# BBischof/ESRecsys

Measured on AMD Instinct MI355X. Metric: training pairs/sec, higher is better.
Workload: dtype f32; 1 GPU; inbatch: V=1000000 x D=128 fp32 tables, B=8192, sparse Adagrad; score_precision=auto -> f16x2, ids=uniform, parallelism=single

## Files before the change

### esrecsys_amd/csrc/esr_optim.hip

```cpp
#include "esr_common.h"
#include "esr_adam.h"
#include "esr_inbatch_mfma.h"
#include "esr_segment.h"

#include <algorithm>

namespace esr {

enum SegOp { kAdagrad = 0, kSgd = 1, kToDense = 2, kMomentum = 3, kMomentumStep = 4, kMomentumStepLazy = 5, kAdamStepLazy = 6 };
struct NoSegExtra {};
struct MomentumArgs {
  float momentum;
};
struct MomentumLazyArgs {
  float momentum;
  int32_t* last[2];
  int now;
};
template <int OP> struct SegExtraT { using type = NoSegExtra; };
template <> struct SegExtraT<kMomentumStep> { using type = MomentumArgs; };
template <> struct SegExtraT<kMomentumStepLazy> { using type = MomentumLazyArgs; };
template <> struct SegExtraT<kAdamStepLazy> { using type = AdamLazyArgs; };

template <int VEC, int NCH>
__device__ __forceinline__ void param_load(RowRegs<VEC, NCH>& r, const void* table, int dtype, int64_t row, int D,
                                           int lig, int G, int nvec) {
  if (dtype == ESR_F32) {
    row_load(r, (const float*)table + row * D, lig, G, nvec);
  } else {
    const uint16_t* p = (const uint16_t*)table + row * D;
#pragma unroll
    for (int k = 0; k < NCH; ++k) {
      const int c = lig + k * G;
      if (c < nvec) {
        if constexpr (VEC == 4) {
          const uint2 u = *reinterpret_cast<const uint2*>(p + 4 * c);
          r.v[k][0] = __uint_as_float(u.x << 16);
          r.v[k][1] = __uint_as_float(u.x & 0xffff0000u);
          r.v[k][2] = __uint_as_float(u.y << 16);
          r.v[k][3] = __uint_as_float(u.y & 0xffff0000u);
        } else {
          r.v[k][0] = bf16_to_f32(p[c]);
        }
      } else {
#pragma unroll
        for (int e = 0; e < VEC; ++e) r.v[k][e] = 0.f;
      }
    }
  }
}

template <int VEC, int NCH>
__device__ __forceinline__ void param_store(const RowRegs<VEC, NCH>& r, void* table, int dtype, int64_t row, int D,
                                            int lig, int G, int nvec) {
  if (dtype == ESR_F32) {
    row_store(r, (float*)table + row * D, lig, G, nvec);
  } else {
    uint16_t* p = (uint16_t*)table + row * D;
#pragma unroll
    for (int k = 0; k < NCH; ++k) {
      const int c = lig + k * G;
      if (c < nvec) {
        if constexpr (VEC == 4) {
          uint2 u;
          u.x = (uint32_t)f32_to_bf16(r.v[k][0]) | ((uint32_t)f32_to_bf16(r.v[k][1]) << 16);
          u.y = (uint32_t)f32_to_bf16(r.v[k][2]) | ((uint32_t)f32_to_bf16(r.v[k][3]) << 16);
          *reinterpret_cast<uint2*>(p + 4 * c) = u;
        } else {
          p[c] = f32_to_bf16(r.v[k][0]);
        }
      }
    }
  }
}

__device__ __forceinline__ void momentum_step_elem(float& p, float& t, float g, float lr, float m) {
#pragma clang fp contract(off)
  t = g + m * t;
  p = p - lr * t;
}

template <int VEC, int NCH, int OP>
__device__ __forceinline__ void seg_apply(const FusedTables& ft, int dtype, int32_t vid, const RowRegs<VEC, NCH>& g,
                                          int D, int lig, int G, int nvec, float lr, float eps,
                                          const typename SegExtraT<OP>::type& ex) {
  void* table = ft.table[0];
  float* accum = ft.accum[0];
  int64_t base = ft.row_offset[0];
#pragma unroll
  for (int k = 1; k < kMaxFusedTables; ++k)
    if (k < ft.n && (int64_t)vid >= ft.row_offset[k]) {
      table = ft.table[k];
      accum = ft.accum[k];
      base = ft.row_offset[k];
    }
  const int64_t id = (int64_t)vid - base;
  const bool second = 1 < ft.n && (int64_t)vid >= ft.row_offset[1];
  if constexpr (OP == kToDense) {
    row_store(g, (float*)table + id * D, lig, G, nvec);
  } else if constexpr (OP == kAdamStepLazy) {
    float* nu = second ? ex.nu[1] : ex.nu[0];
    int32_t* last = second ? ex.last[1] : ex.last[0];
    RowRegs<VEC, NCH> w, a, b;
    row_load(w, (const float*)table + id * D, lig, G, nvec);
    row_load(a, accum + id * D, lig, G, nvec);
    row_load(b, nu + id * D, lig, G, nvec);
    adam_catchup(w, a, b, last[id], ex.now - 1, ex, lig, G);
    const float omb1 = 1.0f - ex.b1, omb2 = 1.0f - ex.b2;
    const int64_t V = (second ? ft.row_offset[2] : ft.row_offset[1]) - base;
#pragma unroll
    for (int k = 0; k < NCH; ++k)
#pragma unroll
      for (int e = 0; e < VEC; ++e) {
        if (VEC == 1 && adam_is_tail(id * D + lig + k * G, V, D))
          adam_elem_tail(w.v[k][e], a.v[k][e], b.v[k][e], g.v[k][e], ex.lr, ex.b1, ex.b2, omb1, omb2, ex.eps, ex.ibc1[0],
                         ex.ibc2[0]);
        else
          adam_elem(w.v[k][e], a.v[k][e], b.v[k][e], g.v[k][e], ex.lr, ex.b1, ex.b2, omb1, omb2, ex.eps, ex.ibc1[0],
                    ex.ibc2[0]);
      }
    row_store(w, (float*)table + id * D, lig, G, nvec);
    row_store(a, accum + id * D, lig, G, nvec);
    row_store(b, nu + id * D, lig, G, nvec);
    if (lig == 0) last[id] = ex.now;
  } else {
    constexpr bool kLazy = OP == kMomentumStepLazy, kState = OP != kSgd;
    int32_t* last = nullptr;
    int steps = 0;
    if constexpr (kLazy) {
      last = second ? ex.last[1] : ex.last[0];
      steps = ex.now - 1 - last[id];
    }
    RowRegs<VEC, NCH> w, a;
    param_load(w, table, dtype, id, D, lig, G, nvec);
    if constexpr (kState) row_load(a, accum + id * D, lig, G, nvec);
    DecayCoef dk{};
    if constexpr (kLazy) dk = decay_coef(steps, ex.momentum);
#pragma unroll
    for (int k = 0; k < NCH; ++k)
#pragma unroll
      for (int e = 0; e < VEC; ++e) {
        float& p = w.v[k][e];
        const float gv = g.v[k][e];
        if constexpr (OP == kSgd) {
          p -= lr * gv;
        } else if constexpr (OP == kMomentum) {
          a.v[k][e] += gv;
          p -= lr * gv;
        } else if constexpr (OP == kAdagrad) {
          adagrad_elem(p, a.v[k][e], gv, lr, eps);
        } else {
          if constexpr (kLazy)
            if (steps > 0) decay_apply(p, a.v[k][e], dk, lr, ex.momentum);
          momentum_step_elem(p, a.v[k][e], gv, lr, ex.momentum);
        }
      }
    if constexpr (kState) row_store(a, accum + id * D, lig, G, nvec);
    param_store(w, table, dtype, id, D, lig, G, nvec);
    if constexpr (kLazy)
      if (lig == 0) last[id] = ex.now;
  }
}

template <int VEC, int NCH, int OP>
__global__ __launch_bounds__(kBlock) void segment_update_kernel(FusedTables ft, int dtype, int D, int G,
                                                               const int32_t* __restrict__ sorted_ids,
                                                               const int32_t* __restrict__ perm, int64_t n,
                                                               float* __restrict__ grad_rows, float lr, float eps,
                                                               typename SegExtraT<OP>::type ex) {
  const int lig = threadIdx.x & (G - 1);
  const int64_t gpb = kBlock / G;
  const int64_t group = (int64_t)blockIdx.x * gpb + threadIdx.x / G;
  const int64_t ngroups = (int64_t)gridDim.x * gpb;
  const int nvec = D / VEC;
  const int64_t per = (n + ngroups - 1) / ngroups;
  const int64_t p_end = min(n, (group + 1) * per);
  for (int64_t p = group * per; p < p_end; ++p) {
    const int32_t id = sorted_ids[p];
    const bool head = p == 0 || sorted_ids[p - 1] != id;
    if (!head && ((p & (kSegChunk - 1)) != 0 || sorted_ids[p - kSegChunk] != id)) continue;
    const int64_t stop = min(head ? ((p + 2 * kSegChunk - 1) / kSegChunk) * kSegChunk : p + kSegChunk, n);
    RowRegs<VEC, NCH> g;
    row_load(g, grad_rows + (int64_t)perm[p] * D, lig, G, nvec);
    int64_t q = p + 1, e_run = p + 1;
    bool run_over = false;
    while (e_run < stop) {
      if (sorted_ids[e_run] != id) {
        run_over = true;
        break;
      }
      ++e_run;
    }
    for (; q + 4 <= e_run; q += 4) {
      RowRegs<VEC, NCH> t0, t1, t2, t3;
      row_load(t0, grad_rows + (int64_t)perm[q] * D, lig, G, nvec);
      row_load(t1, grad_rows + (int64_t)perm[q + 1] * D, lig, G, nvec);
      row_load(t2, grad_rows + (int64_t)perm[q + 2] * D, lig, G, nvec);
      row_load(t3, grad_rows + (int64_t)perm[q + 3] * D, lig, G, nvec);
#pragma unroll
      for (int k = 0; k < NCH; ++k)
#pragma unroll
        for (int e = 0; e < VEC; ++e) g.v[k][e] = (((g.v[k][e] + t0.v[k][e]) + t1.v[k][e]) + t2.v[k][e]) + t3.v[k][e];
    }
    for (; q < e_run; ++q) {
      RowRegs<VEC, NCH> t;
      row_load(t, grad_rows + (int64_t)perm[q] * D, lig, G, nvec);
#pragma unroll
      for (int k = 0; k < NCH; ++k)
#pragma unroll
        for (int e = 0; e < VEC; ++e) g.v[k][e] += t.v[k][e];
    }
    const bool ends = run_over || q == n || sorted_ids[q] != id;
    if (head && ends)
      seg_apply<VEC, NCH, OP>(ft, dtype, id, g, D, lig, G, nvec, lr, eps, ex);
    else
      row_store(g, grad_rows + (int64_t)perm[p] * D, lig, G, nvec);
  }
}

template <int VEC, int NCH, int OP>
__global__ __launch_bounds__(kBlock) void segment_long_kernel(FusedTables ft, int dtype, int D, int G,
                                                             const int32_t* __restrict__ sorted_ids,
                                                             const int32_t* __restrict__ perm, int64_t n,
                                                             const float* __restrict__ grad_rows, float lr,
                                                             float eps, typename SegExtraT<OP>::type ex) {
  __shared__ float red[kBlock * VEC * NCH];
  constexpr int kPass = 4;
  __shared__ long long s_long[kPass];
  __shared__ int s_nlong, s_hoff;
  const int tid = threadIdx.x, lig = tid & (G - 1), gidx = tid / G, NG = kBlock / G;
  const int nvec = D / VEC;
  const int64_t nbound = (n - 1) / kSegChunk;
  for (int64_t b0 = (int64_t)blockIdx.x * kPass; b0 < nbound; b0 += (int64_t)gridDim.x * kPass) {
    __syncthreads();
    if (tid == 0) s_nlong = 0;
    __syncthreads();
    {
      const int64_t B = (b0 + tid + 1) * kSegChunk;
      if (tid < kPass && b0 + tid < nbound) {
        const int32_t id_b = sorted_ids[B];
        const bool first = B < 2 * kSegChunk || sorted_ids[B - 2 * kSegChunk] != id_b;
        if (sorted_ids[B - kSegChunk] == id_b && first) s_long[atomicAdd(&s_nlong, 1)] = B;
      }
    }
    __syncthreads();
    const int nlong = s_nlong;
    for (int li = 0; li < nlong; ++li) {
      const int64_t nxt = s_long[li];
      const int32_t id = sorted_ids[nxt];
      const int64_t win = max<int64_t>(nxt - 2 * kSegChunk + 1, 0);
      if (tid < 64) {
        const int64_t pos = win + tid;
        const bool is_head = pos <= nxt - kSegChunk && sorted_ids[pos] == id && (pos == 0 || sorted_ids[pos - 1] != id);
        const unsigned long long m = __ballot(is_head);
        if (tid == 0) s_hoff = __ffsll((long long)m) - 1;
      }
      __syncthreads();
      const int64_t h = win + s_hoff;
      int64_t K = 0;
      for (int64_t k0 = 0;; k0 += kBlock) {
        const int64_t pos = nxt + (k0 + tid) * kSegChunk;
        const int cnt = __syncthreads_count(pos < n && sorted_ids[pos] == id);
        K += cnt;
        if (cnt < kBlock) break;
      }
      RowRegs<VEC, NCH> acc;
#pragma unroll
      for (int k = 0; k < NCH; ++k)
#pragma unroll
        for (int e = 0; e < VEC; ++e) acc.v[k][e] = 0.f;
      auto part_row = [&](int64_t i) { return (int64_t)perm[i == 0 ? h : nxt + (i - 1) * kSegChunk] * D; };
      int64_t i = gidx;
      for (; i + 3 * NG <= K; i += 4 * NG) {
        RowRegs<VEC, NCH> t0, t1, t2, t3;
        row_load(t0, grad_rows + part_row(i), lig, G, nvec);
        row_load(t1, grad_rows + part_row(i + NG), lig, G, nvec);
        row_load(t2, grad_rows + part_row(i + 2 * NG), lig, G, nvec);
        row_load(t3, grad_rows + part_row(i + 3 * NG), lig, G, nvec);
#pragma unroll
        for (int k = 0; k < NCH; ++k)
#pragma unroll
          for (int e = 0; e < VEC; ++e)
            acc.v[k][e] = (((acc.v[k][e] + t0.v[k][e]) + t1.v[k][e]) + t2.v[k][e]) + t3.v[k][e];
      }
      for (; i <= K; i += NG) {
        RowRegs<VEC, NCH> t;
        row_load(t, grad_rows + part_row(i), lig, G, nvec);
#pragma unroll
        for (int k = 0; k < NCH; ++k)
#pragma unroll
          for (int e = 0; e < VEC; ++e) acc.v[k][e] += t.v[k][e];
      }
#pragma unroll
      for (int k = 0; k < NCH; ++k)
#pragma unroll
        for (int e = 0; e < VEC; ++e) red[((gidx * G + lig) * NCH + k) * VEC + e] = acc.v[k][e];
      __syncthreads();
      if (gidx == 0) {
        const int used = (int)min<int64_t>(NG, K + 1);
        for (int gg = 1; gg < used; ++gg)
#pragma unroll
          for (int k = 0; k < NCH; ++k)
#pragma unroll
            for (int e = 0; e < VEC; ++e) acc.v[k][e] += red[((gg * G + lig) * NCH + k) * VEC + e];
        seg_apply<VEC, NCH, OP>(ft, dtype, id, acc, D, lig, G, nvec, lr, eps, ex);
      }
      __syncthreads();
    }
  }
}

__global__ __launch_bounds__(kBlock) void gather_rows_multi_kernel(FusedTables ft, int nchunk, int G,
                                                                  const int32_t* __restrict__ vids, int64_t n,
                                                                  uint4* __restrict__ out) {
  const int lig = threadIdx.x & (G - 1);
  const int64_t gpb = kBlock / G;
  const int64_t group = (int64_t)blockIdx.x * gpb + threadIdx.x / G;
  const int64_t ngroups = (int64_t)gridDim.x * gpb;
  for (int64_t r = group; r < n; r += ngroups) {
    const int64_t vid = vids[r];
    const uint4* table = reinterpret_cast<const uint4*>(ft.table[0]);
    int64_t base = ft.row_offset[0];
#pragma unroll
    for (int k = 1; k < kMaxFusedTables; ++k)
      if (k < ft.n && vid >= ft.row_offset[k]) {
        table = reinterpret_cast<const uint4*>(ft.table[k]);
        base = ft.row_offset[k];
      }
    const uint4* src = table + (vid - base) * nchunk;
    for (int c = lig; c < nchunk; c += G) out[r * nchunk + c] = src[c];
  }
}

struct IdSegments {
  const int32_t* ids[kMaxFusedTables];
  int64_t start[kMaxFusedTables + 1];
  int64_t offset[kMaxFusedTables];
  int n;
};
__global__ __launch_bounds__(kBlock) void concat_offset_ids_kernel(IdSegments sg, int32_t* __restrict__ out) {
  const int64_t total = sg.start[sg.n];
  for (int64_t i = (int64_t)blockIdx.x * kBlock + threadIdx.x; i < total; i += (int64_t)gridDim.x * kBlock) {
    const int32_t* src = sg.ids[0];
    int64_t start = 0, off = sg.offset[0];
#pragma unroll
    for (int k = 1; k < kMaxFusedTables; ++k)
      if (k < sg.n && i >= sg.start[k]) {
        src = sg.ids[k];
        start = sg.start[k];
        off = sg.offset[k];
      }
    out[i] = (int32_t)((int64_t)src[i - start] + off);
  }
}

template <int OP>
static int launch_segment_tables(const char* who, const FusedTables& ft, int dtype, int D, const int32_t* sorted_ids,
                                 const int32_t* perm, int64_t n, float* grad_rows, float lr, float eps,
                                 hipStream_t st, bool skip_long = false,
                                 typename SegExtraT<OP>::type ex = {}) {
  const RowGeom g = row_geom(D);
  if (g.nch > kMaxChunksPerLane) {
    set_error("%s: D=%d not supported", who, D);
    return ESR_EINVAL;
  }
  const int grid = grid_for_groups(n, g.G);
  const int grid2 = (int)std::min<int64_t>(kMaxGrid, cdiv(cdiv(n, kSegChunk), 4));
  ESR_DISPATCH_ROW(g, {
    ESR_KT("segment_update_kernel", st, hipLaunchKernelGGL((segment_update_kernel<VEC, NCH, OP>), dim3(grid), dim3(kBlock), 0, st, ft, dtype, D, g.G,
                       sorted_ids, perm, n, grad_rows, lr, eps, ex));
    if (n > kSegChunk && !skip_long)
      ESR_KT("segment_long_kernel", st, hipLaunchKernelGGL((segment_long_kernel<VEC, NCH, OP>), dim3(grid2), dim3(kBlock), 0, st, ft, dtype, D, g.G,
                         sorted_ids, perm, n, (const float*)grad_rows, lr, eps, ex));
  });
  return check_launch(who);
}

template <class T>
static int fused_tables(const char* who, FusedTables& ft, T* const* tables, float* const* states,
                        const int64_t* row_offsets, int ntables, bool strict = false, int max_tables = kMaxFusedTables) {
  ESR_REQUIRE(ntables >= 1 && ntables <= max_tables, "%s: ntables=%d not in [1, %d]", who, ntables, max_tables);
  ESR_REQUIRE(tables && row_offsets, "%s: null pointer", who);
  ft.n = ntables;
  for (int i = 0; i < kMaxFusedTables; ++i) {
    ft.table[i] = i < ntables ? const_cast<void*>((const void*)tables[i]) : nullptr;
    ft.accum[i] = i < ntables && states ? states[i] : nullptr;
    ft.row_offset[i] = row_offsets[std::min(i, ntables)];
    if (i < ntables) {
      ESR_REQUIRE(tables[i] || states, "%s: null table %d", who, i);
      ESR_REQUIRE(tables[i] && (!states || states[i]) && row_offsets[i + 1] >= row_offsets[i] + (strict ? 1 : 0),
                  "%s: bad table %d", who, i);
    }
  }
  ft.row_offset[kMaxFusedTables] = row_offsets[ntables];
  ESR_REQUIRE(row_offsets[ntables] < ((int64_t)1 << 31), "%s: %lld virtual rows >= 2^31", who, (long long)row_offsets[ntables]);
  return ESR_OK;
}

template <int OP>
static int launch_segment_update(const char* who, void* table, int dtype, float* accum, int D,
                                 const int32_t* sorted_ids, const int32_t* perm, int64_t n, float* grad_rows,
                                 float lr, float eps, hipStream_t st, typename SegExtraT<OP>::type ex = {}) {
  const int64_t row_offsets[2] = {0, 0};
  FusedTables ft;
  if (const int rc = fused_tables(who, ft, &table, accum ? &accum : nullptr, row_offsets, 1)) return rc;
  return launch_segment_tables<OP>(who, ft, dtype, D, sorted_ids, perm, n, grad_rows, lr, eps, st, false, ex);
}

__global__ __launch_bounds__(kBlock) void dense_adam_kernel(float* __restrict__ p, float* __restrict__ mu,
                                                           float* __restrict__ nu, const float* __restrict__ g,
                                                           int64_t n4, int64_t numel, float lr, float b1, float b2,
                                                           float eps, float inv_bc1, float inv_bc2) {
  const float omb1 = 1.0f - b1, omb2 = 1.0f - b2;
  auto upd = [&](float& pv, float& m, float& v, float gv) {
    adam_elem(pv, m, v, gv, lr, b1, b2, omb1, omb2, eps, inv_bc1, inv_bc2);
  };
  const int64_t stride = (int64_t)gridDim.x * kBlock;
  for (int64_t i = (int64_t)blockIdx.x * kBlock + threadIdx.x; i < n4; i += stride) {
    float4 pv = reinterpret_cast<float4*>(p)[i];
    float4 m = reinterpret_cast<float4*>(mu)[i];
    float4 v = reinterpret_cast<float4*>(nu)[i];
    const float4 gv = reinterpret_cast<const float4*>(g)[i];
    upd(pv.x, m.x, v.x, gv.x);
    upd(pv.y, m.y, v.y, gv.y);
    upd(pv.z, m.z, v.z, gv.z);
    upd(pv.w, m.w, v.w, gv.w);
    reinterpret_cast<float4*>(p)[i] = pv;
    reinterpret_cast<float4*>(mu)[i] = m;
    reinterpret_cast<float4*>(nu)[i] = v;
  }
  for (int64_t i = n4 * 4 + (int64_t)blockIdx.x * kBlock + threadIdx.x; i < numel; i += stride) {
    float pv = p[i], m = mu[i], v = nu[i];
    adam_elem_tail(pv, m, v, g[i], lr, b1, b2, omb1, omb2, eps, inv_bc1, inv_bc2);
    p[i] = pv;
    mu[i] = m;
    nu[i] = v;
  }
}

__global__ __launch_bounds__(kBlock) void momentum_decay_kernel(float* __restrict__ p, float* __restrict__ tr,
                                                               int64_t n4, int64_t numel, float lr, float momentum) {
  const int64_t stride = (int64_t)gridDim.x * kBlock;
  for (int64_t i = (int64_t)blockIdx.x * kBlock + threadIdx.x; i < n4; i += stride) {
    float4 pv = reinterpret_cast<float4*>(p)[i];
    float4 t = reinterpret_cast<float4*>(tr)[i];
    t.x *= momentum; t.y *= momentum; t.z *= momentum; t.w *= momentum;
    pv.x -= lr * t.x; pv.y -= lr * t.y; pv.z -= lr * t.z; pv.w -= lr * t.w;
    reinterpret_cast<float4*>(p)[i] = pv;
    reinterpret_cast<float4*>(tr)[i] = t;
  }
  for (int64_t i = n4 * 4 + (int64_t)blockIdx.x * kBlock + threadIdx.x; i < numel; i += stride) {
    const float t = tr[i] * momentum;
    tr[i] = t;
    p[i] -= lr * t;
  }
}


struct CatchupTables {
  float* table[2];
  float* trace[2];
  int32_t* last[2];
  const int32_t* ids[2];
  int modulus[2];
};

template <int VEC, int NCH>
__global__ __launch_bounds__(kBlock) void momentum_catchup_kernel(CatchupTables ct, int D, int G, int64_t n, int now,
                                                                 float lr, float m) {
  const int y = blockIdx.y;
  float* __restrict__ table = y ? ct.table[1] : ct.table[0];
  float* __restrict__ trace = y ? ct.trace[1] : ct.trace[0];
  int32_t* __restrict__ last = y ? ct.last[1] : ct.last[0];
  const int32_t* __restrict__ ids = y ? ct.ids[1] : ct.ids[0];
  const int modulus = y ? ct.modulus[1] : ct.modulus[0];
  const int lig = threadIdx.x & (G - 1);
  const int64_t gpb = kBlock / G;
  const int nvec = D / VEC;
  for (int64_t i = (int64_t)blockIdx.x * gpb + threadIdx.x / G; i < n; i += (int64_t)gridDim.x * gpb) {
    const int32_t row = modulus > 0 ? ids[i] % modulus : ids[i];
    int old = 0;
    if (lig == 0) old = atomicExch(&last[row], now);
    old = __shfl(old, (threadIdx.x & 63) & ~(G - 1), kWave);
    const int steps = now - 1 - old;
    if (steps <= 0) continue;
    RowRegs<VEC, NCH> w, a;
    row_load(w, table + (int64_t)row * D, lig, G, nvec);
    row_load(a, trace + (int64_t)row * D, lig, G, nvec);
    const DecayCoef dk = decay_coef(steps, m);
#pragma unroll
    for (int k = 0; k < NCH; ++k)
#pragma unroll
      for (int e = 0; e < VEC; ++e) decay_apply(w.v[k][e], a.v[k][e], dk, lr, m);
    row_store(w, table + (int64_t)row * D, lig, G, nvec);
    row_store(a, trace + (int64_t)row * D, lig, G, nvec);
  }
}

template <int VEC, int NCH>
__global__ __launch_bounds__(kBlock) void momentum_flush_kernel(float* __restrict__ table, float* __restrict__ trace,
                                                               int32_t* __restrict__ last, int64_t V, int D, int G,
                                                               int now, float lr, float m) {
  const int lig = threadIdx.x & (G - 1);
  const int64_t gpb = kBlock / G;
  const int nvec = D / VEC;
  for (int64_t row = (int64_t)blockIdx.x * gpb + threadIdx.x / G; row < V; row += (int64_t)gridDim.x * gpb) {
    const int steps = now - last[row];
    if (steps <= 0) continue;
    RowRegs<VEC, NCH> w, a;
    row_load(w, table + row * D, lig, G, nvec);
    row_load(a, trace + row * D, lig, G, nvec);
    const DecayCoef dk = decay_coef(steps, m);
#pragma unroll
    for (int k = 0; k < NCH; ++k)
#pragma unroll
      for (int e = 0; e < VEC; ++e) decay_apply(w.v[k][e], a.v[k][e], dk, lr, m);
    row_store(w, table + row * D, lig, G, nvec);
    row_store(a, trace + row * D, lig, G, nvec);
    if (lig == 0) last[row] = now;
  }
}

}

using namespace esr;

extern "C" {

int esr_momentum_catchup_rows(float* table, float* trace, int32_t* last, int64_t V, int D, const int32_t* ids, int64_t n,
                              int modulus, int step, float lr, float momentum, esr_stream_t stream) {
  ESR_REQUIRE(V > 0 && D > 0 && n >= 0 && step >= 1 && modulus >= 0, "esr_momentum_catchup_rows: bad arguments");
  if (n == 0) return ESR_OK;
  ESR_REQUIRE(table && trace && last && ids, "esr_momentum_catchup_rows: null pointer");
  const RowGeom g = row_geom(D);
  ESR_REQUIRE(g.nch <= kMaxChunksPerLane, "esr_momentum_catchup_rows: D=%d not supported", D);
  const int grid = grid_for_groups(n, g.G);
  CatchupTables ct{{table, nullptr}, {trace, nullptr}, {last, nullptr}, {ids, nullptr}, {modulus, 0}};
  ESR_DISPATCH_ROW(g, hipLaunchKernelGGL((momentum_catchup_kernel<VEC, NCH>), dim3(grid, 1), dim3(kBlock), 0,
                                         as_stream(stream), ct, D, g.G, n, step, lr, momentum));
  return check_launch("esr_momentum_catchup_rows");
}

int esr_momentum_catchup_rows2(float* table0, float* trace0, int32_t* last0, const int32_t* ids0, int modulus0,
                               float* table1, float* trace1, int32_t* last1, const int32_t* ids1, int modulus1, int D,
                               int64_t n, int step, float lr, float momentum, esr_stream_t stream) {
  ESR_REQUIRE(D > 0 && n >= 0 && step >= 1 && modulus0 >= 0 && modulus1 >= 0, "esr_momentum_catchup_rows2: bad arguments");
  if (n == 0) return ESR_OK;
  ESR_REQUIRE(table0 && trace0 && last0 && ids0 && table1 && trace1 && last1 && ids1,
              "esr_momentum_catchup_rows2: null pointer");
  const RowGeom g = row_geom(D);
  ESR_REQUIRE(g.nch <= kMaxChunksPerLane, "esr_momentum_catchup_rows2: D=%d not supported", D);
  const int grid = grid_for_groups(n, g.G);
  CatchupTables ct{{table0, table1}, {trace0, trace1}, {last0, last1}, {ids0, ids1}, {modulus0, modulus1}};
  ESR_DISPATCH_ROW(g, hipLaunchKernelGGL((momentum_catchup_kernel<VEC, NCH>), dim3(grid, 2), dim3(kBlock), 0,
                                         as_stream(stream), ct, D, g.G, n, step, lr, momentum));
  return check_launch("esr_momentum_catchup_rows2");
}

int esr_sparse_momentum_step_multi(float* const* tables, float* const* traces, const int64_t* row_offsets, int ntables,
                                   int D, const int32_t* sorted_vids, const int32_t* perm, int64_t n, float* grad_rows,
                                   float lr, float momentum, esr_stream_t stream) {
  ESR_REQUIRE(ntables >= 1 && ntables <= kMaxFusedTables && D > 0 && n >= 0,
              "esr_sparse_momentum_step_multi: ntables=%d not in [1, %d] or bad sizes", ntables, kMaxFusedTables);
  if (n == 0) return ESR_OK;
  ESR_REQUIRE(tables && traces && row_offsets && sorted_vids && perm && grad_rows,
              "esr_sparse_momentum_step_multi: null pointer");
  FusedTables ft;
  if (const int rc = fused_tables("esr_sparse_momentum_step_multi", ft, tables, traces, row_offsets, ntables))
    return rc;
  return launch_segment_tables<kMomentumStep>("esr_sparse_momentum_step_multi", ft, ESR_F32, D, sorted_vids, perm, n,
                                              grad_rows, lr, 0.f, as_stream(stream), false, {momentum});
}

}

namespace esr {
int sparse_adagrad_range(void* const* tables, float* const* accums, const int64_t* row_offsets, int ntables, int dtype,
                         int D, const int32_t* sorted_vids, const int32_t* perm, int64_t n, float* grad_rows, float lr,
                         float eps, bool skip_long, hipStream_t st) {
  if (!(ntables >= 1 && ntables <= kMaxFusedTables && D > 0 && n >= 0)) {
    set_error("sparse_adagrad_range: bad arguments");
    return ESR_EINVAL;
  }
  if (n == 0) return ESR_OK;
  FusedTables ft;
  if (const int rc = fused_tables("sparse_adagrad_range", ft, tables, accums, row_offsets, ntables)) return rc;
  return launch_segment_tables<kAdagrad>("sparse_adagrad_range", ft, dtype, D, sorted_vids, perm, n, grad_rows, lr, eps, st,
                                         skip_long);
}

template <bool QSIDE>
__device__ __forceinline__ float4 merged_occurrence(const InbatchMergeArgs& a, int64_t r, float4 x, float oscale, int lig,
                                                    float& row_loss) {
  constexpr int side = QSIDE ? 0 : 1;
  const int nsplit = a.nsplit[side];
  float pm[8], pl[8];
  float4 po[8];
#pragma unroll
  for (int s = 0; s < 8; ++s) {
    pm[s] = -INFINITY; pl[s] = 0.f; po[s] = make_float4(0.f, 0.f, 0.f, 0.f);
    if (s < nsplit) {
      if (QSIDE) {
        pm[s] = a.part_m[(int64_t)s * a.B + r];
        pl[s] = a.part_l[(int64_t)s * a.B + r];
      }
      po[s] = *reinterpret_cast<const float4*>(a.part_O[side] + ((int64_t)s * a.B + r) * k3D + 4 * lig);
    }
  }
  const float4 y = *reinterpret_cast<const float4*>(a.partner[side] + r * k3D + 4 * lig);
  float M, L, invL1, wt[8];
  return merge_row<QSIDE>(po, pm, pl, nsplit, false, x, y, oscale, a.scale, a.lam, a.inv_bs, 32, row_loss, M, L, invL1, wt);
}

__global__ __launch_bounds__(kBlock) void inbatch_merge_update_kernel(FusedTables ft, int dtype,
                                                                     const int32_t* __restrict__ sorted_ids,
                                                                     const int32_t* __restrict__ perm, int64_t n,
                                                                     InbatchMergeArgs a, float lr, float eps) {
  constexpr int G = 32, D = k3D, nvec = k3D / 4;
  __shared__ long long sm[4];
  if (a.zero_words && blockIdx.x == 0)
    for (int i = threadIdx.x; i < a.nzero; i += kBlock) a.zero_words[i] = 0ull;
  const int lig = threadIdx.x & (G - 1);
  const int64_t gpb = kBlock / G;
  const int64_t group = (int64_t)blockIdx.x * gpb + threadIdx.x / G;
  const int64_t ngroups = (int64_t)gridDim.x * gpb;
  const int64_t per = (n + ngroups - 1) / ngroups;
  const int64_t p_end = min(n, (group + 1) * per);
  const float osc_q = a.oscale[0][0], osc_c = a.oscale[1][0];
  long long acc_loss = 0;
  bool bad = false;
  for (int64_t p = group * per; p < p_end; ++p) {
    const int32_t vid = sorted_ids[p];
    const bool head = p == 0 || sorted_ids[p - 1] != vid;
    if (!head) {
      if ((p & (kSegChunk - 1)) == 0 && p >= kSegChunk && sorted_ids[p - kSegChunk] == vid) bad = true;
      continue;
    }
    const int64_t stop = min(((p + 2 * kSegChunk - 1) / kSegChunk) * kSegChunk, n);
    void* table = ft.table[0];
    float* accum = ft.accum[0];
    const bool qside = (int64_t)vid < ft.row_offset[1];
    int64_t id = vid;
    if (!qside) {
      table = ft.table[1];
      accum = ft.accum[1];
      id = (int64_t)vid - ft.row_offset[1];
    }
    RowRegs<4, 1> w, ac;
    param_load(w, table, dtype, id, D, lig, G, nvec);
    row_load(ac, accum + id * D, lig, G, nvec);
    const float4 x = make_float4(w.v[0][0], w.v[0][1], w.v[0][2], w.v[0][3]);
    float4 g = make_float4(0.f, 0.f, 0.f, 0.f);
    for (int64_t q = p; q < stop; ++q) {
      if (q > p && sorted_ids[q] != vid) break;
      const int64_t o = perm[q];
      float row_loss;
      const float4 t = qside ? merged_occurrence<true>(a, o, x, osc_q, lig, row_loss)
                             : merged_occurrence<false>(a, o - a.B, x, osc_c, lig, row_loss);
      if (q == p) {
        g = t;
      } else {
        float4 tt = t;
        asm volatile("" : "+v"(tt.x), "+v"(tt.y), "+v"(tt.z), "+v"(tt.w));
        g.x += tt.x; g.y += tt.y; g.z += tt.z; g.w += tt.w;
      }
      if (lig == 0) acc_loss += loss_fixed(row_loss, bad);
      if (q + 1 == stop && q + 1 < n && sorted_ids[q + 1] == vid) bad = true;
    }
    adagrad_elem(w.v[0][0], ac.v[0][0], g.x, lr, eps);
    adagrad_elem(w.v[0][1], ac.v[0][1], g.y, lr, eps);
    adagrad_elem(w.v[0][2], ac.v[0][2], g.z, lr, eps);
    adagrad_elem(w.v[0][3], ac.v[0][3], g.w, lr, eps);
    row_store(ac, accum + id * D, lig, G, nvec);
    param_store(w, table, dtype, id, D, lig, G, nvec);
  }
  const long long tsum = block_sum_ll(acc_loss, sm);
  const bool any_bad = __syncthreads_or(bad ? 1 : 0) != 0;
  if (threadIdx.x == 0) loss_arrive(tsum, any_bad, 1, a.loss_acc, a.loss_scale, a.loss_out);
}

int inbatch_merge_update(void* const* tables, float* const* accums, const int64_t* row_offsets, int dtype,
                         const int32_t* sorted_vids, const int32_t* perm, const InbatchMergeArgs& a, float lr, float eps,
                         hipStream_t st) {
  FusedTables ft;
  if (const int rc = fused_tables("inbatch_merge_update", ft, tables, accums, row_offsets, 2)) return rc;
  const int64_t n = 2 * a.B;
  const int grid = n >= 4096 ? std::max(1, grid_for_groups(n, 32) / 2) : grid_for_groups(n, 32);
  ESR_KT("inbatch_merge_update_kernel", st,
         hipLaunchKernelGGL(inbatch_merge_update_kernel, dim3(grid), dim3(kBlock), 0, st, ft, dtype, sorted_vids, perm, n, a,
                            lr, eps));
  return check_launch("inbatch_merge_update");
}

int sparse_momentum_step_lazy2(float* const* tables, float* const* traces, int32_t* const* lasts, const int64_t* row_offsets,
                               int ntables, int D, const int32_t* sorted_vids, const int32_t* perm, int64_t n, float* grad_rows,
                               float lr, float momentum, int now, hipStream_t st) {
  if (!(ntables >= 1 && ntables <= 2 && D > 0 && n >= 0 && now >= 1)) {
    set_error("sparse_momentum_step_lazy2: ntables=%d not in [1, 2] or bad sizes", ntables);
    return ESR_EINVAL;
  }
  if (n == 0) return ESR_OK;
  FusedTables ft;
  if (const int rc = fused_tables("sparse_momentum_step_lazy2", ft, tables, traces, row_offsets, ntables, false, 2))
    return rc;
  const MomentumLazyArgs ex{momentum, {lasts[0], ntables > 1 ? lasts[1] : nullptr}, now};
  return launch_segment_tables<kMomentumStepLazy>("sparse_momentum_step_lazy2", ft, ESR_F32, D, sorted_vids, perm, n,
                                                  grad_rows, lr, 0.f, st, false, ex);
}
}

extern "C" {

int esr_momentum_flush(float* table, float* trace, int32_t* last, int64_t V, int D, int step, float lr, float momentum,
                       esr_stream_t stream) {
  ESR_REQUIRE(V > 0 && D > 0 && step >= 0, "esr_momentum_flush: bad arguments");
  ESR_REQUIRE(table && trace && last, "esr_momentum_flush: null pointer");
  const RowGeom g = row_geom(D);
  ESR_REQUIRE(g.nch <= kMaxChunksPerLane, "esr_momentum_flush: D=%d not supported", D);
  const int grid = grid_for_groups(V, g.G);
  ESR_DISPATCH_ROW(g, hipLaunchKernelGGL((momentum_flush_kernel<VEC, NCH>), dim3(grid), dim3(kBlock), 0, as_stream(stream),
                                         table, trace, last, V, D, g.G, step, lr, momentum));
  return check_launch("esr_momentum_flush");
}

int esr_sparse_momentum_step(float* table, float* trace, int64_t V, int D, const int32_t* sorted_ids,
                             const int32_t* perm, int64_t n, float* grad_rows, float lr, float momentum,
                             esr_stream_t stream) {
  ESR_REQUIRE(V > 0 && D > 0 && n >= 0, "esr_sparse_momentum_step: bad sizes V=%lld D=%d n=%lld", (long long)V, D,
              (long long)n);
  if (n == 0) return ESR_OK;
  ESR_REQUIRE(table && trace && sorted_ids && perm && grad_rows, "esr_sparse_momentum_step: null pointer");
  return launch_segment_update<kMomentumStep>("esr_sparse_momentum_step", table, ESR_F32, trace, D, sorted_ids, perm, n,
                                              grad_rows, lr, 0.f, as_stream(stream), {momentum});
}

int esr_dense_momentum_decay(float* param, float* trace, int64_t count, float lr, float momentum,
                             esr_stream_t stream) {
  ESR_REQUIRE(count >= 0, "esr_dense_momentum_decay: bad count %lld", (long long)count);
  if (count == 0) return ESR_OK;
  ESR_REQUIRE(param && trace, "esr_dense_momentum_decay: null pointer");
  ESR_REQUIRE((((uintptr_t)param | (uintptr_t)trace) & 15) == 0, "esr_dense_momentum_decay: pointers must be 16-byte aligned");
  const int64_t n4 = count / 4;
  const int grid = (int)std::min<int64_t>(std::max<int64_t>(cdiv(n4, kBlock), 1), 8192);
  hipLaunchKernelGGL(momentum_decay_kernel, dim3(grid), dim3(kBlock), 0, as_stream(stream), param, trace, n4, count, lr,
                     momentum);
  return check_launch("esr_dense_momentum_decay");
}

int esr_sparse_momentum_scatter(float* table, float* trace, int64_t V, int D, const int32_t* sorted_ids,
                                const int32_t* perm, int64_t n, float* grad_rows, float lr,
                                esr_stream_t stream) {
  ESR_REQUIRE(V > 0 && D > 0 && n >= 0, "esr_sparse_momentum_scatter: bad sizes V=%lld D=%d n=%lld", (long long)V, D,
              (long long)n);
  if (n == 0) return ESR_OK;
  ESR_REQUIRE(table && trace && sorted_ids && perm && grad_rows, "esr_sparse_momentum_scatter: null pointer");
  return launch_segment_update<kMomentum>("esr_sparse_momentum_scatter", table, ESR_F32, trace, D, sorted_ids, perm, n,
                                          grad_rows, lr, 0.f, as_stream(stream));
}

int esr_sparse_adagrad_scatter(void* table, int dtype, float* accum, int64_t V, int D, const int32_t* sorted_ids,
                               const int32_t* perm, int64_t n, float* grad_rows, float lr, float eps,
                               esr_stream_t stream) {
  ESR_REQUIRE(V > 0 && D > 0 && n >= 0, "esr_sparse_adagrad_scatter: bad sizes V=%lld D=%d n=%lld", (long long)V, D,
              (long long)n);
  ESR_REQUIRE(dtype == ESR_F32 || dtype == ESR_BF16, "esr_sparse_adagrad_scatter: bad dtype %d", dtype);
  if (n == 0) return ESR_OK;
  ESR_REQUIRE(table && accum && sorted_ids && perm && grad_rows, "esr_sparse_adagrad_scatter: null pointer");
  return launch_segment_update<kAdagrad>("esr_sparse_adagrad_scatter", table, dtype, accum, D, sorted_ids, perm, n,
                                         grad_rows, lr, eps, as_stream(stream));
}

int esr_sparse_sgd_scatter(void* table, int dtype, int64_t V, int D, const int32_t* sorted_ids, const int32_t* perm,
                           int64_t n, float* grad_rows, float lr, esr_stream_t stream) {
  ESR_REQUIRE(V > 0 && D > 0 && n >= 0, "esr_sparse_sgd_scatter: bad sizes V=%lld D=%d n=%lld", (long long)V, D,
              (long long)n);
  ESR_REQUIRE(dtype == ESR_F32 || dtype == ESR_BF16, "esr_sparse_sgd_scatter: bad dtype %d", dtype);
  if (n == 0) return ESR_OK;
  ESR_REQUIRE(table && sorted_ids && perm && grad_rows, "esr_sparse_sgd_scatter: null pointer");
  return launch_segment_update<kSgd>("esr_sparse_sgd_scatter", table, dtype, nullptr, D, sorted_ids, perm, n,
                                     grad_rows, lr, 0.f, as_stream(stream));
}

int esr_rows_to_dense(float* dense, int64_t V, int D, const int32_t* sorted_ids, const int32_t* perm, int64_t n,
                      float* grad_rows, esr_stream_t stream) {
  ESR_REQUIRE(V > 0 && D > 0 && n >= 0, "esr_rows_to_dense: bad sizes V=%lld D=%d n=%lld", (long long)V, D,
              (long long)n);
  ESR_REQUIRE(dense, "esr_rows_to_dense: null pointer");
  hipStream_t st = as_stream(stream);
  if (hipMemsetAsync(dense, 0, sizeof(float) * (size_t)V * D, st) != hipSuccess)
    return check_launch("esr_rows_to_dense memset");
  if (n == 0) return ESR_OK;
  ESR_REQUIRE(sorted_ids && perm && grad_rows, "esr_rows_to_dense: null pointer");
  return launch_segment_update<kToDense>("esr_rows_to_dense", dense, ESR_F32, nullptr, D, sorted_ids, perm, n,
                                         grad_rows, 0.f, 0.f, st);
}

int esr_segment_sum_rows(float* out, int64_t rows_out, int D, const int32_t* sorted_ids, const int32_t* perm, int64_t n,
                         float* grad_rows, esr_stream_t stream) {
  ESR_REQUIRE(rows_out > 0 && D > 0 && n >= 0, "esr_segment_sum_rows: bad sizes rows=%lld D=%d n=%lld", (long long)rows_out,
              D, (long long)n);
  if (n == 0) return ESR_OK;
  ESR_REQUIRE(out && sorted_ids && perm && grad_rows, "esr_segment_sum_rows: null pointer");
  return launch_segment_update<kToDense>("esr_segment_sum_rows", out, ESR_F32, nullptr, D, sorted_ids, perm, n, grad_rows,
                                         0.f, 0.f, as_stream(stream));
}

int esr_concat_offset_ids(const int32_t* const* ids, const int64_t* counts, const int64_t* offsets, int nseg,
                          int32_t* out, esr_stream_t stream) {
  ESR_REQUIRE(nseg >= 1 && nseg <= kMaxFusedTables, "esr_concat_offset_ids: nseg=%d not in [1, %d]", nseg,
              kMaxFusedTables);
  ESR_REQUIRE(ids && counts && offsets && out, "esr_concat_offset_ids: null pointer");
  IdSegments sg;
  sg.n = nseg;
  sg.start[0] = 0;
  for (int i = 0; i < kMaxFusedTables; ++i) {
    sg.ids[i] = i < nseg ? ids[i] : nullptr;
    sg.offset[i] = i < nseg ? offsets[i] : 0;
    sg.start[i + 1] = sg.start[i] + (i < nseg ? counts[i] : 0);
    if (i < nseg) {
      ESR_REQUIRE(counts[i] >= 0 && (counts[i] == 0 || ids[i]), "esr_concat_offset_ids: bad segment %d", i);
    }
  }
  const int64_t total = sg.start[nseg];
  if (total == 0) return ESR_OK;
  const int grid = (int)std::min<int64_t>(kMaxGrid, cdiv(total, kBlock));
  hipLaunchKernelGGL(concat_offset_ids_kernel, dim3(grid), dim3(kBlock), 0, as_stream(stream), sg, out);
  return check_launch("esr_concat_offset_ids");
}

int esr_gather_rows_multi(const void* const* tables, const int64_t* row_offsets, int ntables, int dtype, int D,
                          const int32_t* vids, int64_t n, void* out, esr_stream_t stream) {
  ESR_REQUIRE(ntables >= 1 && ntables <= kMaxFusedTables, "esr_gather_rows_multi: ntables=%d not in [1, %d]", ntables,
              kMaxFusedTables);
  ESR_REQUIRE(dtype == ESR_F32 || dtype == ESR_BF16, "esr_gather_rows_multi: bad dtype %d", dtype);
  ESR_REQUIRE(D > 0 && n >= 0, "esr_gather_rows_multi: bad sizes D=%d n=%lld", D, (long long)n);
  const int64_t row_bytes = (int64_t)D * (dtype == ESR_BF16 ? 2 : 4);
  ESR_REQUIRE(row_bytes % 16 == 0, "esr_gather_rows_multi: row of %lld bytes is not a multiple of 16", (long long)row_bytes);
  if (n == 0) return ESR_OK;
  ESR_REQUIRE(tables && row_offsets && vids && out, "esr_gather_rows_multi: null pointer");
  FusedTables ft;
  if (const int rc = fused_tables("esr_gather_rows_multi", ft, tables, nullptr, row_offsets, ntables)) return rc;
  const int nchunk = (int)(row_bytes / 16);
  int G = 1;
  while (G < nchunk && G < kWave) G <<= 1;
  const int grid = grid_for_groups(n, G);
  hipLaunchKernelGGL(gather_rows_multi_kernel, dim3(grid), dim3(kBlock), 0, as_stream(stream), ft, nchunk, G, vids, n,
                     (uint4*)out);
  return check_launch("esr_gather_rows_multi");
}

__global__ __launch_bounds__(kBlock) void long_run_hint_kernel(const int32_t* __restrict__ sorted_ids, int64_t n, int chunk,
                                                              int* __restrict__ hint, int gen) {
  bool long_run = false;
  for (int64_t p = (int64_t)blockIdx.x * kBlock + threadIdx.x; p + chunk < n; p += (int64_t)gridDim.x * kBlock)
    if (sorted_ids[p] == sorted_ids[p + chunk]) long_run = true;
  if (__any(long_run) && (threadIdx.x & 63) == 0) hint[0] = gen;
}

int esr_long_run_hint(const int32_t* sorted_ids, int64_t n, int chunk, int32_t* hint, int32_t gen, esr_stream_t stream) {
  ESR_REQUIRE(n >= 0 && chunk > 0 && hint && (n == 0 || sorted_ids), "esr_long_run_hint: bad arguments");
  if (n <= chunk) return ESR_OK;
  const int grid = (int)std::min<int64_t>(kMaxGrid, cdiv(n, kBlock));
  hipLaunchKernelGGL(long_run_hint_kernel, dim3(grid), dim3(kBlock), 0, as_stream(stream), sorted_ids, n, chunk, hint, gen);
  return check_launch("esr_long_run_hint");
}

int esr_sparse_adagrad_scatter_multi(void* const* tables, float* const* accums, const int64_t* row_offsets,
                                     int ntables, int dtype, int D, const int32_t* sorted_vids, const int32_t* perm,
                                     int64_t n, float* grad_rows, float lr, float eps, int long_runs,
                                     esr_stream_t stream) {
  TraceScope trace_scope_("esr_sparse_adagrad_scatter_multi");
  ESR_REQUIRE(ntables >= 1 && ntables <= kMaxFusedTables, "esr_sparse_adagrad_scatter_multi: ntables=%d not in [1, %d]",
              ntables, kMaxFusedTables);
  ESR_REQUIRE(D > 0 && n >= 0, "esr_sparse_adagrad_scatter_multi: bad sizes D=%d n=%lld", D, (long long)n);
  ESR_REQUIRE(dtype == ESR_F32 || dtype == ESR_BF16, "esr_sparse_adagrad_scatter_multi: bad dtype %d", dtype);
  if (n == 0) return ESR_OK;
  ESR_REQUIRE(tables && accums && row_offsets && sorted_vids && perm && grad_rows,
              "esr_sparse_adagrad_scatter_multi: null pointer");
  FusedTables ft;
  if (const int rc = fused_tables("esr_sparse_adagrad_scatter_multi", ft, tables, accums, row_offsets, ntables)) return rc;
  return launch_segment_tables<kAdagrad>("esr_sparse_adagrad_scatter_multi", ft, dtype, D, sorted_vids, perm, n,
                                         grad_rows, lr, eps, as_stream(stream), long_runs == 0);
}

int esr_sparse_adam_step_lazy(float* const* tables, float* const* mus, float* const* nus, int32_t* const* lasts,
                              const int64_t* row_offsets, int ntables, int D, const int32_t* sorted_vids, const int32_t* perm,
                              int64_t n, float* grad_rows, float lr, float b1, float b2, float eps, int step,
                              esr_stream_t stream) {
  ESR_REQUIRE(ntables >= 1 && ntables <= 2 && D > 0 && n >= 0 && step >= 1,
              "esr_sparse_adam_step_lazy: ntables=%d not in [1, 2] or bad D=%d n=%lld step=%d", ntables, D, (long long)n, step);
  ESR_REQUIRE(row_geom(D).nch <= kMaxChunksPerLane, "esr_sparse_adam_step_lazy: D=%d not supported", D);
  ESR_REQUIRE(tables && mus && nus && lasts && row_offsets && sorted_vids && perm && grad_rows,
              "esr_sparse_adam_step_lazy: null pointer");
  ESR_REQUIRE((((uintptr_t)sorted_vids | (uintptr_t)perm) & 3) == 0 && ((uintptr_t)grad_rows & 15) == 0,
              "esr_sparse_adam_step_lazy: misaligned ids or gradient rows");
  FusedTables ft;
  if (const int rc = fused_tables("esr_sparse_adam_step_lazy", ft, tables, mus, row_offsets, ntables, true, 2))
    return rc;
  AdamLazyArgs ax;
  adam_lazy_args(ax, lr, b1, b2, eps, step);
  for (int i = 0; i < ntables; ++i) {
    ESR_REQUIRE(nus[i] && lasts[i], "esr_sparse_adam_step_lazy: bad table %d", i);
    ESR_REQUIRE((((uintptr_t)tables[i] | (uintptr_t)mus[i] | (uintptr_t)nus[i]) & 15) == 0 && ((uintptr_t)lasts[i] & 3) == 0,
                "esr_sparse_adam_step_lazy: table %d: pointers must be 16-byte aligned", i);
    ax.nu[i] = nus[i];
    ax.last[i] = lasts[i];
  }
  ESR_REQUIRE(row_offsets[0] == 0, "esr_sparse_adam_step_lazy: row_offsets[0] must be 0");
  if (n == 0) return ESR_OK;
  return launch_segment_tables<kAdamStepLazy>("esr_sparse_adam_step_lazy", ft, ESR_F32, D, sorted_vids, perm, n, grad_rows,
                                              lr, eps, as_stream(stream), false, ax);
}

int esr_dense_adam(float* param, float* mu, float* nu, const float* grad, int64_t numel, float lr, float b1,
                   float b2, float eps, int64_t step, esr_stream_t stream) {
  ESR_REQUIRE(numel >= 0 && step >= 1, "esr_dense_adam: bad numel=%lld step=%lld", (long long)numel, (long long)step);
  if (numel == 0) return ESR_OK;
  ESR_REQUIRE(param && mu && nu && grad, "esr_dense_adam: null pointer");
  ESR_REQUIRE((((uintptr_t)param | (uintptr_t)mu | (uintptr_t)nu | (uintptr_t)grad) & 15) == 0,
              "esr_dense_adam: pointers must be 16-byte aligned");
  const double bc1 = 1.0 - pow((double)b1, (double)step);
  const double bc2 = 1.0 - pow((double)b2, (double)step);
  const int64_t n4 = numel / 4;
  const int grid = (int)std::min<int64_t>(kMaxGrid, std::max<int64_t>(1, cdiv(n4, kBlock)));
  hipLaunchKernelGGL(dense_adam_kernel, dim3(grid), dim3(kBlock), 0, as_stream(stream), param, mu, nu, grad, n4,
                     numel, lr, b1, b2, eps, (float)(1.0 / bc1), (float)(1.0 / bc2));
  return check_launch("esr_dense_adam");
}

}
```

Baseline: 39.93 million pairs/s.

## Restructure inbatch merge-update loop with windowed head search and batched occurrence loads

Rewrites the fused merge+Adagrad kernel's per-group loop. Each lane now loads 32 sorted ids and perms at once and finds segment heads with a ballot, replacing per-position scalar global reads. All loads for an occurrence (partials, partner, m/l values via one lane-distributed load plus shuffles, and the weight and accumulator rows) are issued together before the merge math. The kernel is templated on dtype so the dtype branches compile away. This adds control-flow complexity, extra speculative loads (weight rows re-read for non-head occurrences, partials loaded for every split slot), and a slightly different grid sizing computation.

```diff
diff --git a/esrecsys_amd/csrc/esr_optim.hip b/esrecsys_amd/csrc/esr_optim.hip
--- a/esrecsys_amd/csrc/esr_optim.hip
+++ b/esrecsys_amd/csrc/esr_optim.hip
@@ -589,8 +589,36 @@
                                          skip_long);
 }
 
+struct OccLoads {
+  float4 po[8];
+  float4 y;
+  float ml;
+  RowRegs<4, 1> w, ac;
+};
+
+template <bool BF16>
+__device__ __forceinline__ void occ_issue(OccLoads& ld, const FusedTables& ft, const InbatchMergeArgs& a, int32_t vid,
+                                          int32_t o, int lig) {
+  constexpr int G = 32, D = k3D, nvec = k3D / 4, dtype = BF16 ? ESR_BF16 : ESR_F32;
+  const bool qside = (int64_t)vid < ft.row_offset[1];
+  void* const table = qside ? ft.table[0] : ft.table[1];
+  const float* const accum = qside ? ft.accum[0] : ft.accum[1];
+  const int64_t id = qside ? (int64_t)vid : (int64_t)vid - ft.row_offset[1];
+  param_load(ld.w, table, dtype, id, D, lig, G, nvec);
+  row_load(ld.ac, accum + id * D, lig, G, nvec);
+  const int64_t r = qside ? (int64_t)o : (int64_t)o - a.B;
+  const float* const part = qside ? a.part_O[0] : a.part_O[1];
+  const int last = max((qside ? a.nsplit[0] : a.nsplit[1]) - 1, 0);
+#pragma unroll
+  for (int s = 0; s < 8; ++s)
+    ld.po[s] = *reinterpret_cast<const float4*>(part + ((int64_t)min(s, last) * a.B + r) * k3D + 4 * lig);
+  ld.y = *reinterpret_cast<const float4*>((qside ? a.partner[0] : a.partner[1]) + r * k3D + 4 * lig);
+  const float* const ml = (lig & 8) ? a.part_l : a.part_m;
+  ld.ml = ml[(int64_t)min(lig & 7, max(a.nsplit[0] - 1, 0)) * a.B + (qside ? r : 0)];
+}
+
 template <bool QSIDE>
-__device__ __forceinline__ float4 merged_occurrence(const InbatchMergeArgs& a, int64_t r, float4 x, float oscale, int lig,
+__device__ __forceinline__ float4 merged_occurrence(const InbatchMergeArgs& a, const OccLoads& ld, float4 x, float oscale,
                                                     float& row_loss) {
   constexpr int side = QSIDE ? 0 : 1;
   const int nsplit = a.nsplit[side];
@@ -599,24 +627,23 @@
 #pragma unroll
   for (int s = 0; s < 8; ++s) {
     pm[s] = -INFINITY; pl[s] = 0.f; po[s] = make_float4(0.f, 0.f, 0.f, 0.f);
-    if (s < nsplit) {
-      if (QSIDE) {
-        pm[s] = a.part_m[(int64_t)s * a.B + r];
-        pl[s] = a.part_l[(int64_t)s * a.B + r];
-      }
-      po[s] = *reinterpret_cast<const float4*>(a.part_O[side] + ((int64_t)s * a.B + r) * k3D + 4 * lig);
-    }
-  }
-  const float4 y = *reinterpret_cast<const float4*>(a.partner[side] + r * k3D + 4 * lig);
+    if (QSIDE) {
+      const float m = __shfl(ld.ml, s, 32), l = __shfl(ld.ml, 8 + s, 32);
+      if (s < nsplit) { pm[s] = m; pl[s] = l; }
+    }
+    if (s < nsplit) po[s] = ld.po[s];
+  }
   float M, L, invL1, wt[8];
-  return merge_row<QSIDE>(po, pm, pl, nsplit, false, x, y, oscale, a.scale, a.lam, a.inv_bs, 32, row_loss, M, L, invL1, wt);
-}
-
-__global__ __launch_bounds__(kBlock) void inbatch_merge_update_kernel(FusedTables ft, int dtype,
+  return merge_row<QSIDE>(po, pm, pl, nsplit, false, x, ld.y, oscale, a.scale, a.lam, a.inv_bs, 32, row_loss, M, L, invL1,
+                          wt);
+}
+
+template <bool BF16>
+__global__ __launch_bounds__(kBlock) void inbatch_merge_update_kernel(FusedTables ft,
                                                                      const int32_t* __restrict__ sorted_ids,
                                                                      const int32_t* __restrict__ perm, int64_t n,
                                                                      InbatchMergeArgs a, float lr, float eps) {
-  constexpr int G = 32, D = k3D, nvec = k3D / 4;
+  constexpr int G = 32, D = k3D, nvec = k3D / 4, dtype = BF16 ? ESR_BF16 : ESR_F32;
   __shared__ long long sm[4];
   if (a.zero_words && blockIdx.x == 0)
     for (int i = threadIdx.x; i < a.nzero; i += kBlock) a.zero_words[i] = 0ull;
@@ -629,50 +656,98 @@
   const float osc_q = a.oscale[0][0], osc_c = a.oscale[1][0];
   long long acc_loss = 0;
   bool bad = false;
-  for (int64_t p = group * per; p < p_end; ++p) {
-    const int32_t vid = sorted_ids[p];
-    const bool head = p == 0 || sorted_ids[p - 1] != vid;
-    if (!head) {
-      if ((p & (kSegChunk - 1)) == 0 && p >= kSegChunk && sorted_ids[p - kSegChunk] == vid) bad = true;
-      continue;
-    }
-    const int64_t stop = min(((p + 2 * kSegChunk - 1) / kSegChunk) * kSegChunk, n);
-    void* table = ft.table[0];
-    float* accum = ft.accum[0];
+  const int p0 = (int)min(n, group * per), pe = (int)p_end, nn = (int)n;
+  const int half = threadIdx.x & 32;
+
+  int wb = p0;
+  int32_t sid_l = 0, prm_l = 0;
+  uint32_t heads = 0;
+  auto load_window = [&](int base) {
+    wb = base;
+    const int pos = base + lig, cp = min(pos, nn - 1);
+    sid_l = sorted_ids[cp];
+    prm_l = perm[cp];
+    const int32_t left = sorted_ids[max(cp - 1, 0)];
+    const bool head = pos < nn && (pos == 0 || left != sid_l);
+    const bool cont = pos < pe && !head && (pos & (kSegChunk - 1)) == 0 && pos >= kSegChunk;
+    if (sorted_ids[cont ? pos - kSegChunk : cp] == sid_l && cont) bad = true;
+    heads = (uint32_t)(__ballot(head) >> half);
+  };
+  auto find_head = [&](int pos) -> int {
+    while (pos < pe) {
+      if (pos - wb >= G) load_window(pos);
+      const uint32_t m = heads >> (pos - wb);
+      if (m) return min(pos + __builtin_ctz(m), pe);
+      pos = wb + G;
+    }
+    return pe;
+  };
+
+  int q = pe, run_stop = 0;
+  int32_t vid = 0;
+  bool cur_head = true;
+  RowRegs<4, 1> w, ac;
+  float4 g = make_float4(0.f, 0.f, 0.f, 0.f);
+  const auto chunk_stop = [&](int p) { return (int)min(((int64_t)p + 2 * kSegChunk - 1) / kSegChunk * kSegChunk, n); };
+  auto finish = [&](const OccLoads& cur, bool more) {
+    if (cur_head) {
+      w = cur.w;
+      ac = cur.ac;
+    }
     const bool qside = (int64_t)vid < ft.row_offset[1];
-    int64_t id = vid;
-    if (!qside) {
-      table = ft.table[1];
-      accum = ft.accum[1];
-      id = (int64_t)vid - ft.row_offset[1];
-    }
-    RowRegs<4, 1> w, ac;
-    param_load(w, table, dtype, id, D, lig, G, nvec);
-    row_load(ac, accum + id * D, lig, G, nvec);
     const float4 x = make_float4(w.v[0][0], w.v[0][1], w.v[0][2], w.v[0][3]);
-    float4 g = make_float4(0.f, 0.f, 0.f, 0.f);
-    for (int64_t q = p; q < stop; ++q) {
-      if (q > p && sorted_ids[q] != vid) break;
-      const int64_t o = perm[q];
-      float row_loss;
-      const float4 t = qside ? merged_occurrence<true>(a, o, x, osc_q, lig, row_loss)
-                             : merged_occurrence<false>(a, o - a.B, x, osc_c, lig, row_loss);
-      if (q == p) {
-        g = t;
-      } else {
-        float4 tt = t;
-        asm volatile("" : "+v"(tt.x), "+v"(tt.y), "+v"(tt.z), "+v"(tt.w));
-        g.x += tt.x; g.y += tt.y; g.z += tt.z; g.w += tt.w;
-      }
-      if (lig == 0) acc_loss += loss_fixed(row_loss, bad);
-      if (q + 1 == stop && q + 1 < n && sorted_ids[q + 1] == vid) bad = true;
-    }
-    adagrad_elem(w.v[0][0], ac.v[0][0], g.x, lr, eps);
-    adagrad_elem(w.v[0][1], ac.v[0][1], g.y, lr, eps);
-    adagrad_elem(w.v[0][2], ac.v[0][2], g.z, lr, eps);
-    adagrad_elem(w.v[0][3], ac.v[0][3], g.w, lr, eps);
-    row_store(ac, accum + id * D, lig, G, nvec);
-    param_store(w, table, dtype, id, D, lig, G, nvec);
+    float row_loss;
+    const float4 t = qside ? merged_occurrence<true>(a, cur, x, osc_q, row_loss)
+                           : merged_occurrence<false>(a, cur, x, osc_c, row_loss);
+    if (cur_head) {
+      g = t;
+    } else {
+      float4 tt = t;
+      asm volatile("" : "+v"(tt.x), "+v"(tt.y), "+v"(tt.z), "+v"(tt.w));
+      g.x += tt.x; g.y += tt.y; g.z += tt.z; g.w += tt.w;
+    }
+    if (lig == 0) acc_loss += loss_fixed(row_loss, bad);
+    if (!more) {
+      void* const table = qside ? ft.table[0] : ft.table[1];
+      float* const accum = qside ? ft.accum[0] : ft.accum[1];
+      const int64_t id = qside ? (int64_t)vid : (int64_t)vid - ft.row_offset[1];
+      adagrad_elem(w.v[0][0], ac.v[0][0], g.x, lr, eps);
+      adagrad_elem(w.v[0][1], ac.v[0][1], g.y, lr, eps);
+      adagrad_elem(w.v[0][2], ac.v[0][2], g.z, lr, eps);
+      adagrad_elem(w.v[0][3], ac.v[0][3], g.w, lr, eps);
+      row_store(ac, accum + id * D, lig, G, nvec);
+      param_store(w, table, dtype, id, D, lig, G, nvec);
+    }
+  };
+  if (p0 < pe) {
+    load_window(p0);
+    q = find_head(p0);
+  }
+  if (q < pe) {
+    vid = __shfl(sid_l, q - wb, G);
+    int32_t o = __shfl(prm_l, q - wb, G);
+    run_stop = chunk_stop(q);
+    for (;;) {
+      OccLoads cur;
+      occ_issue<BF16>(cur, ft, a, vid, o, lig);
+      const int nq = q + 1;
+      bool more = false;
+      if (nq < nn) {
+        if (nq - wb >= G) load_window(nq);
+        if (__shfl(sid_l, nq - wb, G) == vid) {
+          if (nq < run_stop) more = true;
+          else bad = true;
+        }
+      }
+      const int nx = more ? nq : find_head(nq);
+      finish(cur, more);
+      if (!more && nx >= pe) break;
+      q = nx;
+      vid = __shfl(sid_l, nx - wb, G);
+      o = __shfl(prm_l, nx - wb, G);
+      cur_head = !more;
+      if (!more) run_stop = chunk_stop(nx);
+    }
   }
   const long long tsum = block_sum_ll(acc_loss, sm);
   const bool any_bad = __syncthreads_or(bad ? 1 : 0) != 0;
@@ -685,10 +760,17 @@
   FusedTables ft;
   if (const int rc = fused_tables("inbatch_merge_update", ft, tables, accums, row_offsets, 2)) return rc;
   const int64_t n = 2 * a.B;
-  const int grid = n >= 4096 ? std::max(1, grid_for_groups(n, 32) / 2) : grid_for_groups(n, 32);
-  ESR_KT("inbatch_merge_update_kernel", st,
-         hipLaunchKernelGGL(inbatch_merge_update_kernel, dim3(grid), dim3(kBlock), 0, st, ft, dtype, sorted_vids, perm, n, a,
-                            lr, eps));
+  const int64_t per = n >= 4096 ? 2 : 1;
+  const int grid = grid_for_groups(cdiv(n, per), 32);
+  if (dtype == ESR_BF16) {
+    ESR_KT("inbatch_merge_update_kernel", st,
+           hipLaunchKernelGGL(inbatch_merge_update_kernel<true>, dim3(grid), dim3(kBlock), 0, st, ft, sorted_vids, perm, n,
+                              a, lr, eps));
+  } else {
+    ESR_KT("inbatch_merge_update_kernel", st,
+           hipLaunchKernelGGL(inbatch_merge_update_kernel<false>, dim3(grid), dim3(kBlock), 0, st, ft, sorted_vids, perm, n,
+                              a, lr, eps));
+  }
   return check_launch("inbatch_merge_update");
 }
 
```

Result: no change. 40.23 million pairs/s, median of 5 (+0.7%).
